# forestagostinelli/DeepCubeA

Hardware: AMD Instinct MI355X
Metric: A* nodes expanded/sec on cube3, batch 20k (higher is better)
Workload: dtype u8 states / f64 cost keys / f32 heuristic

## Files before the change

### deepcubea_amd/csrc/dca_engine.hip

```cpp
#include <string.h>

#include <new>
#include <vector>

#include "dca_common.h"
#include "dca_tile.h"

namespace dca {

constexpr int NBIN = 4096;
constexpr int kBinsPerThread = NBIN / 1024;
constexpr int kLgNbin = 12;
constexpr int kSub = 2048;
constexpr int kScanBlocks = 256;
constexpr int kCollectBlocks = 512;
constexpr int kRankBlocks = 256;
constexpr uint32_t kTinyBin = 512;
constexpr int kSortCap = 8192;
constexpr int RT = 512;
constexpr int kRegEnt = 16;
constexpr uint32_t kLdsEnt = RT * kRegEnt;
constexpr int kStash = 2560;
constexpr int kSegs = NBIN + 1 + kSub;
constexpr uint32_t kGiantBin = 8192;
// ... 1934 lines not shown
                s0[u] = S.off[sub];
                cn[u] = S.off[sub + 1] - s0[u];
                rank[u] = s0[u];
                if (!((livem >> u) & 1u)) cn[u] = 0;
                if (cn[u] > kSubMax && refinable) {
                    bigm |= 1u << u;
                    cn[u] = 0;
                }
                trip = cn[u] > trip ? cn[u] : trip;
            }
            for (uint32_t jj = 0; jj < trip; jj++) {
#pragma unroll
                for (int u = 0; u < U; u++) {
                    const uint32_t j = s0[u] + (jj < cn[u] ? jj : 0u);
                    const bool less = pair_less(LK[j], LI[j], o[u], id[u]);
                    rank[u] += (jj < cn[u] && less) ? 1u : 0u;
                }
            }
            uint32_t retm = 0;
#pragma unroll
            for (int u = 0; u < U; u++) {
                const uint32_t p = p0 + (uint32_t)u * RT + t;
                o[u] = idmode ? kbase : kbase + o[u];
                if ((bigm >> u) & 1u) {
                    K2[p] = o[u];
                    I2[p] = id[u];
                } else if ((livem >> u) & 1u) {
                    if (rank[u] < need) emit_pop(E, c, it.off + rank[u], o[u], id[u]);
                    else retm |= 1u << u;
                }
            }
            ret_put_many<U>(E, S, nf, n_ord, retm, o, id);
        }
        rank_push(S, it, tsub, need, refinable, lo_sub, in_hi);
        __syncthreads();
        prof_end(E, P_RB_ORDER);
        return;
    }
    {
        u128 vmin = ~(u128)0, vmax = 0;
        for (uint32_t b0 = 0; b0 < n; b0 += kLdsEnt) {
            uint64_t ek[kRegEnt];
            uint32_t ei[kRegEnt];
#pragma unroll
            for (int j = 0; j < kRegEnt; j++) {
                const uint32_t i = b0 + t + (uint32_t)RT * j, ic = i < n ? i : n - 1;
                ek[j] = K[ic];
                ei[j] = I[ic];
            }
#pragma unroll
            for (int j = 0; j < kRegEnt; j++)
                if (b0 + t + (uint32_t)RT * j < n) {
                    const u128 v = comp_of(ek[j], ei[j]);
                    vmin = v < vmin ? v : vmin;
                    vmax = v > vmax ? v : vmax;
                }
        }
        rank_range(S, vmin, vmax);
    }
    const u128 base = ((u128)S.vmin_hi << 64) | S.vmin_lo;
    const uint32_t bits = S.bits;
    if (lg > bits) lg = bits;
    const uint32_t nsub = 1u << lg, shc = bits - lg;
    for (uint32_t b0 = 0; b0 < n; b0 += kLdsEnt) {
        uint64_t ek[kRegEnt];
        uint32_t ei[kRegEnt];
#pragma unroll
        for (int j = 0; j < kRegEnt; j++) {
            const uint32_t i = b0 + t + (uint32_t)RT * j, ic = i < n ? i : n - 1;
            ek[j] = K[ic];
            ei[j] = I[ic];
        }
#pragma unroll
        for (int j = 0; j < kRegEnt; j++)
            if (b0 + t + (uint32_t)RT * j < n) atomicAdd(&S.cnt[sub_of(ek[j], ei[j], base, shc, nsub)], 1u);
    }
    __syncthreads();
    rank_prefix(S, nsub, need);
    const uint32_t tsub = S.tsub;
    const bool tsub_pushed = S.off[tsub + 1] - S.off[tsub] > kSubMax && shc > 0;
    ret_begin(c, S, nf, (n - S.off[tsub + 1]) + (tsub_pushed ? 0u : S.off[tsub + 1] - need));
    RetAcc acc{};
    const uint32_t n_ord_all = c->n_ord;
    for (uint32_t b0 = 0; b0 < n; b0 += kLdsEnt) {
        uint64_t ek[kRegEnt];
        uint32_t ei[kRegEnt];
#pragma unroll
        for (int j = 0; j < kRegEnt; j++) {
            const uint32_t i = b0 + t + (uint32_t)RT * j, ic = i < n ? i : n - 1;
            ek[j] = K[ic];
            ei[j] = I[ic];
        }
        uint32_t retm = 0;
#pragma unroll
        for (int j = 0; j < kRegEnt; j++) {
            const bool live = b0 + t + (uint32_t)RT * j < n;
            uint32_t sub = 0;
            if (live) {
                sub = sub_of(ek[j], ei[j], base, shc, nsub);
                if (sub <= tsub) {
                    const uint32_t p = S.off[sub] + atomicAdd(&S.cnt[sub], 1u);
                    K2[p] = ek[j];
                    I2[p] = ei[j];
                }
            }
            retm |= (live && sub > tsub ? 1u : 0u) << j;
        }
        ret_put_many<kRegEnt>(E, S, nf, n_ord_all, retm, ek, ei);
    }
    __syncthreads();
    const uint32_t m = S.off[tsub + 1];
    for (uint32_t p0 = 0; p0 < m; p0 += RT) {
        const uint32_t p = p0 + t;
        bool live = p < m;
        uint64_t k = 0;
        uint32_t id = 0, rank = 0;
        if (live) {
            k = K2[p];
            id = I2[p];
            const uint32_t sub = sub_of(k, id, base, shc, nsub);
            const uint32_t s0 = S.off[sub], e0 = S.off[sub + 1];
            if (e0 - s0 > kSubMax && shc > 0) {
                live = false;
            } else {
                rank = s0;
                for (uint32_t j = s0; j < e0; j++) rank += pair_less(K2[j], I2[j], k, id) ? 1u : 0u;
                if (rank < need) emit_pop(E, c, it.off + rank, k, id);
            }
        }
        ret_put(E, c, S, nf, live && rank >= need, k, id, acc);
    }
    rank_push(S, it, tsub, need, shc > 0);
    ret_end(c, nf, acc);
    __syncthreads();
}

__global__ __launch_bounds__(RT) void k_rank(const Eng* __restrict__ engs) {
    const Eng& E = engs[blockIdx.y];
    gp<Ctl> c = E.ctl;
    if (c->done) return;
    Stamp stamp(E, P_RANK);
    __shared__ RankShared S;
    extern __shared__ __attribute__((aligned(16))) uint8_t rank_lds[];
    uint64_t* LK = reinterpret_cast<uint64_t*>(rank_lds);
    uint32_t* LI = reinterpret_cast<uint32_t*>(rank_lds + (size_t)kLdsEnt * 8);
    const uint32_t t = threadIdx.x;
    const uint32_t nf = c->cur_f;
    const uint32_t tseg = c->tseg, want = c->want;
    const uint32_t n_big = c->n_big, n_ord = c->n_ord;
    if (blockIdx.x == gridDim.x - 1) {
        const uint32_t bstar = c->bstar, pre_b = c->pre_b, cn_star = c->cn_star;
        if (want != 0) {
            for (uint32_t bin = t; bin < bstar; bin += RT) E.hist[bin] = 0;
            if (t == 0) E.hist[bstar] = cn_star - (want - pre_b);
        }
        for (uint32_t i = t; i < (uint32_t)kSegs; i += RT) E.fill[i] = 0;
        if (c->giant)
            for (uint32_t i = t; i < (uint32_t)(kMaxLevels * kSub); i += RT) E.subhist[i] = 0;
    }
    {
        Stamp sub(E, P_RANK_SMALL);
        for (uint32_t p0 = blockIdx.x * RT; p0 < n_ord; p0 += gridDim.x * RT)
            rank_small_entries(E, c, S, LK, LI, nf, p0, n_ord, want);
    }
    Stamp sub2(E, P_RANK_BIG);
    for (uint32_t bi = (blockIdx.x + gridDim.x - 64u) % gridDim.x; bi < n_big; bi += gridDim.x) {
        const uint32_t unit = E.big_list[bi];
        const uint32_t f = unit & 0xFFFFu;
        const uint32_t o = E.pre[f], n = E.pre[f + 1] - o;
        __syncthreads();
        if (t == 0) {
            S.stack[0] = RankItem{o, n, (f == tseg) ? want - o : n, 0u, (unit >> 16) & 15u, unit >> 20, 0u};
            S.sp = 1;
            S.fail = 0;
        }
        for (;;) {
            __syncthreads();
            const uint32_t sp = S.sp;
            if (sp == 0 || sp > (uint32_t)kRankStack) break;
            const RankItem it = S.stack[sp - 1];
            __syncthreads();
            if (t == 0) S.sp = sp - 1;
            __syncthreads();
            rank_item(E, c, S, LK, LI, nf, want, it);
        }
        if (t == 0 && (S.fail || S.sp != 0)) c->failed = 1;
    }
}

__device__ __forceinline__ void close_pop(const Eng& E, gp<Ctl> c, const IterState& S0, uint32_t it, uint32_t want,
                                          uint32_t npop, uint32_t base, bool fail) {
    IterState N = S0;
    if (E.sem == DCA_SEM_PY) {
        const unsigned long long gb = c->goal_best;
        if (gb != ~0ull) {
            c->stop_after = 1;
            c->goal_id = E.pop_id[(uint32_t)(gb & 0xFFFFFFFFull)] & ID_MASK;
        }
    } else {
        const uint32_t fs = c->first_solved;
        if (fs != NIL) {
            const float cst = (float)cost_of_key(E.pop_key[fs]);
            if (E.B == 1) {
                N.best_id = E.pop_id[fs] & ID_MASK;
                N.best_cost = cst;
                N.has_best = 1;
                c->stop_after = 1;
            } else if (!S0.has_best || S0.best_cost > cst) {
                N.best_id = E.pop_id[fs] & ID_MASK;
                N.best_cost = cst;
                N.has_best = 1;
            }
        }
        if (S0.has_best && (float)cost_of_key(E.pop_key[0]) >= N.best_cost) c->stop_after = 1;
    }
    if (fail) {
        c->failed = 1;
        c->done = 1;
        c->front_dead.v -= want;
        return;
    }
    const uint32_t m = npop * (uint32_t)E.A;
    N.npop = npop;
    N.m = m;
    N.base = base;
    N.pool_n = base + m;
    c->S[(it + 1) & 1] = N;
    c->gen += (int64_t)m;
    c->expanded += npop;
}

constexpr uint8_t F_KEEP = 1, F_MIN = 2, F_NEW = 4;

template <int ENV, int DIM>
__device__ __forceinline__ uint32_t child_word_from_parent(uint32_t pw, uint32_t w, uint32_t a, const uint8_t* ltab) {
    using EV = EnvT<ENV, DIM>;
    const int gbase = (int)(threadIdx.x & 63u) & ~15;
    uint32_t out = 0;
    if constexpr (ENV == DCA_ENV_CUBE3) {
#pragma unroll
        for (uint32_t b = 0; b < 4; b++) {
            const uint32_t i = 4 * w + b;
            const uint32_t p = i < (uint32_t)EV::D ? ltab[a * EV::D + i] : 0u;
            const uint32_t v = (uint32_t)__shfl((int)pw, gbase + (int)(p >> 2));
            if (i < (uint32_t)EV::D) out |= ((v >> (8 * (p & 3))) & 0xFFu) << (8 * b);
        }
    } else if constexpr (ENV == DCA_ENV_LIGHTSOUT) {
#pragma unroll
        for (uint32_t b = 0; b < 4; b++) {
            const uint32_t i = 4 * w + b;
            if (i < (uint32_t)EV::D) {
                const uint32_t v = (pw >> (8 * b)) & 0xFFu;
                out |= (lightsout_flip(DIM, (int)a, (int)i) ? ((v + 1u) & 1u) : v) << (8 * b);
            }
        }
    } else {
        uint32_t z = 0xFFFFu;
#pragma unroll
        for (int b = 3; b >= 0; b--)
            if (4 * w + b < (uint32_t)EV::D && ((pw >> (8 * b)) & 0xFFu) == 0u) z = 4 * w + b;
        for (int o = 8; o > 0; o >>= 1) {
            const uint32_t y = (uint32_t)__shfl_xor((int)z, o);
            z = y < z ? y : z;
        }
        z = z < (uint32_t)EV::D ? z : 0u;
        const uint32_t sw = (uint32_t)npuzzle_swap(DIM, (int)z, (int)a);
#pragma unroll
        for (uint32_t b = 0; b < 4; b++) {
            const uint32_t i = 4 * w + b;
            const uint32_t src = i < (uint32_t)EV::D ? ((i == z) ? sw : i) : 0u;
            const uint32_t v = (uint32_t)__shfl((int)pw, gbase + (int)(src >> 2));
            if (i < (uint32_t)EV::D) out |= ((i == sw) ? 0u : ((v >> (8 * (src & 3))) & 0xFFu)) << (8 * b);
        }
    }
    return out;
}

constexpr int kEngTile = 16;
template <int ENV, int DIM, int OH>
__global__ __launch_bounds__(kThreads) void k_expand(const Eng* __restrict__ engs, int heur_id, int write_nn) {
    const Eng& E = engs[blockIdx.y];
    using EV = EnvT<ENV, DIM>;
    using TL = Tile<ENV, DIM, kEngTile>;
    constexpr int kTileParents = kEngTile;
    constexpr int TP = kEngTile;
    typedef uint32_t u32x4 __attribute__((ext_vector_type(4)));
    constexpr int kPermChunks = (int)sizeof(Cube3Perm) / 16;
    u32x4 permv;
    if constexpr (ENV == DCA_ENV_CUBE3) {
        static_assert(sizeof(Cube3Perm) % 16 == 0 && alignof(Cube3Perm) == 16 && TL::TAB_BYTES == (int)sizeof(Cube3Perm),
                      "cube3's move table is staged in 16-byte pieces");
        const u32x4* pp = reinterpret_cast<const u32x4*>(&d_cube3_perm) + min(threadIdx.x, (uint32_t)kPermChunks - 1u);
        asm volatile("global_load_dwordx4 %0, %1, off" : "=v"(permv) : "v"(pp) : "memory");
    }
    gp<Ctl> c = E.ctl;
    if (c->done) return;
    Stamp stamp(E, P_EXPAND);
    extern __shared__ __attribute__((aligned(16))) uint8_t smem[];
    uint8_t* lpar = smem;
    uint8_t* ltab = smem + TL::PAR_BYTES;
    uint8_t* lst = smem + TL::LDS_BYTES;
    __shared__ uint32_t l_pid[TP], l_g[TP], l_mv[TP];
    __shared__ uint32_t l_qn, l_qcc[kThreads], l_qrep[kThreads], l_qres[kThreads];
    __shared__ uint32_t l_ohq;
    const uint32_t it = (uint32_t)c->iters;
    const IterState S0 = c->S[it & 1];
    const uint32_t want = c->want;
    const uint32_t cur_new = c->cur_f;
    uint32_t npop = want;
    if (E.sem == DCA_SEM_CPP) {
        const uint32_t fs = c->first_solved;
        if (fs != NIL) npop = fs + 1;
    }
    const uint32_t base = (S0.pool_n + 15u) & ~15u;
    const bool fail = (uint64_t)base + (uint64_t)npop * (uint64_t)EV::A > (uint64_t)E.max_nodes;
    if (blockIdx.x == 0 && threadIdx.x == 0) close_pop(E, c, S0, it, want, npop, base, fail);
    if (fail) return;
    const uint32_t r0 = blockIdx.x * kTileParents;
    if (E.sem == DCA_SEM_CPP && r0 + kTileParents > npop) {
        uint32_t r = r0 + threadIdx.x;
        bool back = threadIdx.x < kTileParents && r >= npop && r < want;
        open_append(E, c, cur_new, back, back ? E.pop_key[r] : 0, back ? E.pop_id[r] : 0);
        if (back) atomicAdd(&E.hist[bin_of(E.pop_key[r], c->sel_kmin, c->shift)], 1u);
    }
    if (r0 >= npop) return;
    const uint32_t np = min((uint32_t)kTileParents, npop - r0);
    if (OH != 0 && threadIdx.x == 0) l_ohq = 0;
    {
        constexpr int WPR = (EV::D + 3) / 4;
        static_assert(WPR + 2 <= 16, "16 lanes per parent: the row's words, its path cost, its move");
        static_assert(TP * 16 == kThreads, "one 16-lane group per parent of the tile");
        const uint32_t w = threadIdx.x & 15, r = threadIdx.x >> 4;
        gp<const uint32_t> ppop = E.pop_id;
        gp<const uint8_t> pst = E.state, pg = reinterpret_cast<gp<const uint8_t>>(E.g), pmv = E.move;
        asm volatile("" : "+s"(ppop), "+s"(pst), "+s"(pg), "+s"(pmv));
        const uint32_t pid = ppop[r0 + min(r, np - 1u)] & ID_MASK;
        const GatherWord gw = gather_word(EV::D, (int)w);
        const bool row_lane = w < (uint32_t)WPR;
        gp<const uint8_t> src = (row_lane ? pst : pg) + (row_lane ? (size_t)pid * EV::D + (uint32_t)gw.off : (size_t)pid * 4);
        uint32_t v = load_word(src);
        uint32_t mv = pmv[pid];
        asm volatile("" : "+v"(v), "+v"(mv));
        if (r < np) {
            if (w < (uint32_t)WPR) {
                v >>= gw.shift;
                uint8_t* dst = lpar + r * EV::D + 4 * w;
                if constexpr (EV::D % 4 == 0) {
                    *reinterpret_cast<uint32_t*>(dst) = v;
                } else if constexpr (EV::D % 2 == 0) {
                    *reinterpret_cast<uint16_t*>(dst) = (uint16_t)v;
                    if (gw.n == 4) *reinterpret_cast<uint16_t*>(dst + 2) = (uint16_t)(v >> 16);
                } else {
#pragma unroll
                    for (int b = 0; b < 4; b++)
                        if (b < gw.n) dst[b] = (uint8_t)(v >> (8 * b));
                }
            } else if (w == (uint32_t)WPR) {
                l_pid[r] = pid;
                l_g[r] = v;
            } else if (w == (uint32_t)WPR + 1u) {
                l_mv[r] = mv;
            }
        }
    }
    if constexpr (ENV == DCA_ENV_CUBE3) {
        asm volatile("s_waitcnt vmcnt(0)" : "+v"(permv) : : "memory");
        if (threadIdx.x < (uint32_t)kPermChunks) reinterpret_cast<u32x4*>(ltab)[threadIdx.x] = permv;
    }
    __syncthreads();
    if constexpr (ENV != DCA_ENV_CUBE3) {
        stage_tables<ENV, DIM>(ltab, lpar, np);
        __syncthreads();
    }
    TL t{lpar, ltab};
    const uint32_t nchild = np * EV::A;
    const uint32_t j0 = r0 * EV::A;

    auto oh_emit = [&]() {
        if constexpr (OH != 0) {
            constexpr uint32_t ROW = EV::D * EV::DEPTH;
            constexpr uint32_t EPC = 16 / OH;
            const uint32_t te = nchild * ROW;
            const uint32_t one16 = E.oh_dtype == DCA_DT_F16 ? 0x3C00u : 0x3F80u;
            gp<uint8_t> goh = E.onehot + (size_t)j0 * ROW * OH;
            const uint32_t nch = (te + EPC - 1) / EPC;
            auto staged_nnet = [&](uint32_t i) -> uint32_t {
                const uint32_t b = lst[i];
                return ENV == DCA_ENV_CUBE3 ? (b * 57u) >> 9 : b;
            };
            for (;;) {
                uint32_t piece = 0;
                if ((threadIdx.x & 63u) == 0) piece = atomicAdd(&l_ohq, 1u);
                piece = (uint32_t)__builtin_amdgcn_readfirstlane((int)piece);
                if (piece * 64u >= nch) break;
                const uint32_t q = piece * 64u + (threadIdx.x & 63u);
                if (q >= nch) continue;
                uint32_t e0 = q * EPC;
                if constexpr (ENV == DCA_ENV_CUBE3 && OH == 4) {
                    if (e0 + EPC <= te) {
                        const uint32_t P0 = (q << 1) / 3u, phase = (q << 1) - 3u * P0;
                        uint32_t w[4];
                        cube3_onehot32_chunk(phase, staged_nnet(P0), phase == 2u ? staged_nnet(P0 + 1u) : 0u, w);
                        store16(goh + (size_t)e0 * OH, w, true);
                        continue;
                    }
                }
                if constexpr (ENV == DCA_ENV_CUBE3 && OH == 2) {
                    if (e0 + EPC <= te) {
                        const uint32_t P0 = (q << 2) / 3u, phase = (q << 2) - 3u * P0;
                        uint32_t w[4];
                        cube3_onehot16_chunk(phase, staged_nnet(P0), staged_nnet(P0 + 1u), one16, w);
                        store16(goh + (size_t)e0 * OH, w, true);
                        continue;
                    }
                }
                uint32_t cch = e0 / ROW, e = e0 - cch * ROW;
                uint32_t pos = e / EV::DEPTH, col = e - pos * EV::DEPTH;
                uint32_t r = cch / EV::A, a = cch - r * EV::A;
                uint32_t nb = staged_nnet(cch * EV::D + pos);
                uint32_t w[4] = {0, 0, 0, 0};
#pragma unroll
                for (uint32_t k = 0; k < EPC; k++) {
                    bool hot = (nb == col) && (e0 + k < te);
                    if constexpr (OH == 4)
                        w[k] = hot ? 0x3F800000u : 0u;
                    else
                        w[k >> 1] |= (hot ? one16 : 0u) << (16 * (k & 1));
                    if (++col == EV::DEPTH) {
                        col = 0;
                        if (++pos == EV::D) {
                            pos = 0;
                            if (++a == EV::A) {
                                a = 0;
                                ++r;
                            }
                        }
                        nb = staged_nnet((r * EV::A + a) * EV::D + pos);
                    }
                }
                uint8_t* dst = goh + (size_t)e0 * OH;
                if (e0 + EPC <= te) {
                    store16(dst, w, true);
                } else {
                    for (uint32_t k = 0; e0 + k < te; k++) {
                        if constexpr (OH == 4)
                            reinterpret_cast<uint32_t*>(dst)[k] = w[k];
                        else
                            reinterpret_cast<uint16_t*>(dst)[k] = (uint16_t)(w[k >> 1] >> (16 * (k & 1)));
                    }
                }
            }
        }
    };

    if (threadIdx.x == 0) l_qn = 0;
    for (uint32_t cc0 = 0; cc0 < nchild; cc0 += kThreads) {
        const uint32_t cc = cc0 + threadIdx.x;
        const bool cvalid = cc < nchild;
        uint64_t h = 0;
        uint64_t roww[(EV::D + 7) / 8];
        bool known = false;
        if (cvalid) {
        uint32_t r = cc / EV::A, a = cc - r * EV::A;
        static_assert((uint64_t)EV::D * 255u * (7u * (EV::D - 1) + 3u) < (1ull << 32), "the heuristics' byte sum overflows 32 bits");
        static_assert(7 * (EV::D - 1) + 3 < 65536, "the heuristics' weights are two bytes");
        uint32_t sum = 0, sum_hi = 0;
        h = hash_init(EV::D);
        uint32_t manh = 0;
        bool ok = true;
#pragma unroll
        for (int k = 0; k < EV::D; k += 8) {
            uint64_t w = 0;
#pragma unroll
            for (int j = 0; j < 8; j++) {
                if (k + j < EV::D) {
                    uint32_t b = t.child_byte(r, a, k + j);
                    w |= (uint64_t)b << (8 * j);
                    if constexpr (ENV == DCA_ENV_NPUZZLE) manh += manhattan_term(DIM, (uint32_t)(k + j), b);
                }
            }
            h = hash_word(h, w);
            roww[k >> 3] = w;
            ok &= (w & row_word_mask(EV::D, k >> 3)) == goal_word(ENV, EV::D, k >> 3);
#pragma unroll
            for (int q = 0; q < 8; q += 4) {
                if (k + q < EV::D) {
                    const uint32_t x = (uint32_t)(w >> (8 * q));
                    sum = __builtin_amdgcn_udot4(x, sum_weights(k + q, 0), sum, false);
                    if (sum_weights(k + q, 8) != 0u) sum_hi = __builtin_amdgcn_udot4(x, sum_weights(k + q, 8), sum_hi, false);
                }
            }
            uint8_t* dst = lst + cc * EV::D + k;
#pragma unroll
            for (int j = 0; j < 8; j += 2) {
                if (k + j + 1 < EV::D && (EV::D % 2) == 0) {
                    *reinterpret_cast<uint16_t*>(dst + j) = (uint16_t)(w >> (8 * j));
                } else {
                    if (k + j < EV::D) dst[j] = (uint8_t)(w >> (8 * j));
                    if (k + j + 1 < EV::D) dst[j + 1] = (uint8_t)(w >> (8 * j + 8));
                }
            }
        }
        h = hash_final(h);
        const uint32_t j = j0 + cc, id = base + j, pid = l_pid[r];
        const uint32_t gp = l_g[r];
        bool noop = false;
        if constexpr (ENV == DCA_ENV_NPUZZLE) noop = ltab[r * 8 + 1 + a] == ltab[r * 8];
        known = known_duplicate(ENV, gp, l_mv[r], a, noop);
        if (a == 0) E.pop_g[r0 + r] = gp;
        E.g[id] = (int32_t)(gp + 1u);
        E.parent[id] = pid;
        E.move[id] = (uint8_t)a;
        E.solved[id] = ok ? 1 : 0;
        if (heur_id >= 0) E.child_h[j] = heur_from(heur_id, (uint64_t)(sum + (sum_hi << 8)), h, manh);
        }
        {
            constexpr int NWD = (EV::D + 3) / 4;
            const uint32_t j = j0 + cc, id = base + j;
            const uint64_t tag = h >> 32;
            bool active = cvalid && !known, inserted = false, paused = false;
            uint32_t slot = (uint32_t)h & E.tab_mask, v0 = known ? 0u : GINF, rep_id = 0, probes = 0, qi = 0;
            __syncthreads();
            for (;;) {
                if (active && !paused) {
                    for (;;) {
                        const uint4 sl = *reinterpret_cast<const uint4*>(&E.tab[slot]);
                        uint64_t e = ((uint64_t)sl.y << 32) | sl.x;
                        v0 = sl.z;
                        if (e == EMPTY) {
                            const uint64_t old = atomicCAS((unsigned long long*)&E.tab[slot].entry, (unsigned long long)EMPTY,
                                                           (unsigned long long)((tag << 32) | id));
                            if (old == EMPTY) {
                                inserted = true;
                                active = false;
                                break;
                            }
                            e = old;
                        }
                        if ((e >> 32) == tag) {
                            const uint32_t rep = (uint32_t)e;
                            if (rep >= base) {
                                qi = atomicAdd(&l_qn, 1u);
                                l_qcc[qi] = cc;
                                l_qrep[qi] = rep;
                                paused = true;
                                break;
                            }
                            gp<const uint8_t> rrow = E.state + (size_t)rep * EV::D;
                            uint32_t diff = 0;
#pragma unroll
                            for (int k = 0; k < NWD; k++) {
                                uint32_t v = 0;
                                if (4 * k + 4 <= EV::D) {
                                    v = load_word(rrow + 4 * k);
                                } else {
                                    for (int b = 0; 4 * k + b < EV::D; b++) v |= (uint32_t)rrow[4 * k + b] << (8 * b);
                                }
                                diff |= v ^ (uint32_t)(roww[k >> 1] >> (32 * (k & 1)));
                            }
                            if (diff == 0) {
                                rep_id = rep;
                                active = false;
                                break;
                            }
                        }
                        slot = (slot + 1) & E.tab_mask;
                        if (++probes > E.tab_mask) {
                            c->failed = 1;
                            active = false;
                            break;
                        }
                    }
                }
                __syncthreads();
                const uint32_t nq = l_qn;
                if (nq == 0) break;
                for (uint32_t q0 = 0; q0 < nq; q0 += kThreads / 16) {
                    const uint32_t item = q0 + (threadIdx.x >> 4), w = threadIdx.x & 15u;
                    const bool iv = item < nq;
                    const uint32_t itc = iv ? item : 0u;
                    const uint32_t rrel = l_qrep[itc] - base;
                    const uint32_t rk = rrel / (uint32_t)EV::A, a2 = rrel - rk * (uint32_t)EV::A;
                    const uint32_t ppid = E.pop_id[rk] & ID_MASK;
                    gp<const uint8_t> prow = E.state + (size_t)ppid * EV::D;
                    uint32_t pw = 0;
                    if (w < (uint32_t)NWD) {
                        if (4 * w + 4 <= (uint32_t)EV::D) {
                            pw = load_word(prow + 4 * w);
                        } else {
                            for (uint32_t b = 0; 4 * w + b < (uint32_t)EV::D; b++) pw |= (uint32_t)prow[4 * w + b] << (8 * b);
                        }
                    }
                    const uint32_t cw = child_word_from_parent<ENV, DIM>(pw, w, a2, ltab);
                    const uint8_t* mrow = lst + l_qcc[itc] * EV::D;
                    uint32_t mv = 0;
                    for (uint32_t b = 0; b < 4 && 4 * w + b < (uint32_t)EV::D; b++) mv |= (uint32_t)mrow[4 * w + b] << (8 * b);
                    uint32_t diff = w < (uint32_t)NWD ? (cw ^ mv) : 0u;
                    for (int o = 8; o > 0; o >>= 1) diff |= (uint32_t)__shfl_xor((int)diff, o);
                    if (iv && w == 0) l_qres[item] = diff == 0 ? 1u : 0u;
                }
                __syncthreads();
                if (paused) {
                    paused = false;
                    if (l_qres[qi]) {
                        rep_id = l_qrep[qi];
                        active = false;
                    } else {
                        slot = (slot + 1) & E.tab_mask;
                        probes++;
                    }
                }
                __syncthreads();
                if (threadIdx.x == 0) l_qn = 0;
                __syncthreads();
            }
            if (cvalid) {
                uint32_t prev = NIL;
                if (!inserted && !known) {
                    const uint32_t old_head = atomicExch(&E.tab[slot].head, id);
                    if (old_head >= base)
                        prev = old_head - base;
                    else if (rep_id >= base)
                        prev = rep_id - base;
                }
                E.child_next[j] = prev;
                E.child_slot[j] = slot;
                E.child_v0[j] = v0;
                E.child_flags[j] = inserted ? F_NEW : 0;
                if (prev != NIL) {
                    E.child_multi[j] = 1;
                    E.child_multi[prev] = 1;
                }
            }
        }
    }

    __syncthreads();
    if (!write_nn) {
        const uint32_t tb = nchild * EV::D;
        gp<uint8_t> gpool = E.state + ((size_t)base + j0) * EV::D;
        const uint32_t nfull = tb >> 4;
        for (uint32_t q = threadIdx.x; q < nfull; q += kThreads)
            reinterpret_cast<uint4*>(gpool)[q] = reinterpret_cast<const uint4*>(lst)[q];
#pragma unroll 1
        for (uint32_t bq = (nfull << 4) + threadIdx.x; bq < tb; bq += kThreads) gpool[bq] = lst[bq];
    } else {
        const uint32_t tb = nchild * EV::D;
        gp<uint8_t> gpool = E.state + ((size_t)base + j0) * EV::D;
        gp<uint8_t> gnn = E.nnet_in + (size_t)j0 * EV::D;
        const uint32_t nfull = tb >> 4;
        for (uint32_t q = threadIdx.x; q < nfull; q += kThreads) {
            const uint4 v = reinterpret_cast<const uint4*>(lst)[q];
            reinterpret_cast<uint4*>(gpool)[q] = v;
            if constexpr (ENV == DCA_ENV_CUBE3) {
                auto div9 = [](uint32_t x) {
                    uint32_t lo = (((x & 0x00FF00FFu) * 57u) >> 9) & 0x00070007u;
                    uint32_t hi = ((((x >> 8) & 0x00FF00FFu) * 57u) >> 9) & 0x00070007u;
                    return lo | (hi << 8);
                };
                reinterpret_cast<uint4*>(gnn)[q] = make_uint4(div9(v.x), div9(v.y), div9(v.z), div9(v.w));
            } else {
                reinterpret_cast<uint4*>(gnn)[q] = v;
            }
        }
#pragma unroll 1
        for (uint32_t bq = (nfull << 4) + threadIdx.x; bq < tb; bq += kThreads) {
            const uint32_t b = lst[bq];
            gpool[bq] = (uint8_t)b;
            gnn[bq] = (uint8_t)(ENV == DCA_ENV_CUBE3 ? (b * 57u) >> 9 : b);
        }
    }

    oh_emit();
}

struct Dec {
    bool keep, is_min;
    uint32_t first;
};
__device__ __forceinline__ Dec decide_child(const Eng& E, uint32_t base, uint32_t m, uint32_t j, uint32_t slot,
                                            uint32_t v0, uint32_t gj, bool multi) {
    if (!multi) return Dec{gj < v0, true, j};
    bool dominated = false;
    uint32_t gmin = GINF, pmin = NIL, first = j;
    const uint32_t A = (uint32_t)E.A;
    uint32_t steps = 0;
    for (uint32_t k = E.tab[slot].head - base; k < m && steps <= m; k = E.child_next[k], steps++) {
        const uint32_t gk = E.pop_g[k / A] + 1u;
        dominated |= (k < j && gk <= gj);
        if (gk < gmin || (gk == gmin && k < pmin)) {
            gmin = gk;
            pmin = k;
        }
        first = k < first ? k : first;
    }
    return Dec{(gj < v0) && !dominated, j == pmin, first};
}

__device__ __forceinline__ void fix_representative(const Eng& E, uint32_t base, uint32_t slot, uint32_t id) {
    const uint64_t e = E.tab[slot].entry;
    if ((uint32_t)e >= base && (uint32_t)e != id) E.tab[slot].entry = (e & 0xFFFFFFFF00000000ull) | id;
}

__global__ __launch_bounds__(256) void k_decide(const Eng* __restrict__ engs) {
    const Eng& E = engs[blockIdx.y];
    gp<Ctl> c = E.ctl;
    if (c->done) return;
    Stamp stamp(E, P_DECIDE);
    const uint32_t j = blockIdx.x * 256 + threadIdx.x;
    gr<const IterState> S1 = st_next(c);
    const uint32_t m = S1.m, base = S1.base;
    if (j >= m) return;
    const uint32_t slot = E.child_slot[j];
    const bool multi = E.child_multi[j] != 0;
    const uint32_t gj = E.pop_g[j / (uint32_t)E.A] + 1u;
    const Dec d = decide_child(E, base, m, j, slot, E.child_v0[j], gj, multi);
    E.child_flags[j] = (E.child_flags[j] & F_NEW) | (d.keep ? F_KEEP : 0) | (d.is_min ? F_MIN : 0);
    if (multi && j == d.first) fix_representative(E, base, slot, base + j);
}

template <int ENV, int DIM, int OH>
__global__ __launch_bounds__(256) void k_pack(const Eng* __restrict__ engs) {
    const Eng& E = engs[blockIdx.y];
    using EV = EnvT<ENV, DIM>;
    gp<Ctl> c = E.ctl;
    if (c->done) {
        if (blockIdx.x == 0 && threadIdx.x == 0) {
            atomicAdd(&E.pk_n[1], 1u);
            if (c->failed) atomicAdd(&E.pk_n[2], 1u);
        }
        return;
    }
    Stamp stamp(E, P_PACK);
    const uint32_t m = st_next(c).m, base = st_next(c).base;
    if (blockIdx.x * 256 >= m) return;
    __shared__ uint32_t sh[6];
    __shared__ uint32_t lsrc[256];
    __shared__ __attribute__((aligned(16))) uint8_t lrow[256 * EV::D];
    const uint32_t j = blockIdx.x * 256 + threadIdx.x;
    const bool keep = j < m && (E.child_flags[j] & F_KEEP);
    const int lane = threadIdx.x & 63, wv = threadIdx.x >> 6;
    const unsigned long long mask = __ballot(keep);
    if (lane == 0) sh[wv] = (uint32_t)__popcll(mask);
    __syncthreads();
    if (threadIdx.x == 0) {
        uint32_t tot = 0;
        for (int w = 0; w < 4; w++) {
            uint32_t t = sh[w];
            sh[w] = tot;
            tot += t;
        }
        sh[4] = tot;
        sh[5] = tot ? atomicAdd(E.pk_n, tot) : 0u;
    }
    __syncthreads();
    const uint32_t total = sh[4], gbase = sh[5];
    const uint32_t lr = sh[wv] + (uint32_t)__popcll(mask & ((1ull << lane) - 1ull));
    if (j < m) E.kept_pos[j] = keep ? gbase + lr : NIL;
    if (keep) lsrc[lr] = j;
    __syncthreads();
    if (total == 0) return;
    if (threadIdx.x < total) E.pk_src[gbase + threadIdx.x] = E.inst * E.M + lsrc[threadIdx.x];
    const uint32_t tb = total * EV::D;
    for (uint32_t q = threadIdx.x; q < tb; q += 256) {
        const uint32_t r = q / EV::D, b = q - r * EV::D;
        const uint32_t v = E.state[(size_t)(base + lsrc[r]) * EV::D + b];
        lrow[q] = (uint8_t)(ENV == DCA_ENV_CUBE3 ? (v * 57u) >> 9 : v);
    }
    __syncthreads();
    gp<uint8_t> gnn = E.pk_nnet + (size_t)gbase * EV::D;
    for (uint32_t q = threadIdx.x; q < tb; q += 256) gnn[q] = lrow[q];
    if constexpr (OH != 0) {
        constexpr uint32_t ROW = EV::D * EV::DEPTH, EPC = 16 / OH;
        const uint32_t cpr = E.pk_stride / EPC;
        const uint32_t one16 = E.pk_dtype == DCA_DT_F16 ? 0x3C00u : 0x3F80u;
        uint4* goh = reinterpret_cast<uint4*>(E.pk_onehot + (size_t)gbase * E.pk_stride * OH);
        const uint32_t nch = total * cpr;
        for (uint32_t q = threadIdx.x; q < nch; q += 256) {
            const uint32_t r = q / cpr, e0 = (q - r * cpr) * EPC;
            uint32_t pos = e0 / EV::DEPTH, col = e0 - pos * EV::DEPTH;
            uint32_t nb = pos < (uint32_t)EV::D ? lrow[r * EV::D + pos] : 0xFFFFu;
            uint32_t w[4] = {0, 0, 0, 0};
#pragma unroll
            for (uint32_t k = 0; k < EPC; k++) {
                const bool hot = (e0 + k < ROW) && nb == col;
                if constexpr (OH == 4)
                    w[k] = hot ? 0x3F800000u : 0u;
                else
                    w[k >> 1] |= (hot ? one16 : 0u) << (16 * (k & 1));
                if (++col == EV::DEPTH) {
                    col = 0;
                    ++pos;
                    nb = pos < (uint32_t)EV::D ? lrow[r * EV::D + pos] : 0xFFFFu;
                }
            }
            goh[q] = make_uint4(w[0], w[1], w[2], w[3]);
        }
    }
}

__device__ __forceinline__ void commit_ticket(const Eng& E, gp<Ctl> c) {
    __syncthreads();
    if (threadIdx.x == 0) {
        uint32_t t = atomicAdd(&c->ticket_a.v, 1u);
        if (t == gridDim.x - 1) {
            c->ticket_a.v = 0;
            c->iters += 1;
            if (c->stop_after || c->failed) {
                c->done = 1;
            } else {
                const uint32_t fb = c->cur_f;
                const uint32_t live = __hip_atomic_load(&c->open_n[fb].v, __ATOMIC_RELAXED, __HIP_MEMORY_SCOPE_AGENT) -
                                      __hip_atomic_load(&c->front_dead.v, __ATOMIC_RELAXED, __HIP_MEMORY_SCOPE_AGENT) - c->front_above;
                c->want = live < (uint32_t)E.B ? live : (uint32_t)E.B;
                c->ret_n.v = 0;
                c->goal_best = ~0ull;
                c->first_solved = NIL;
                c->gbar.v = 0;
                c->grange.kmin = ~0ull;
                c->grange.kmax = 0;
                c->grange.imin = ~0u;
                c->grange.imax = 0;
            }
        }
    }
// ... 1158 lines not shown
```

### deepcubea_amd/csrc/dca_tile.h

```cpp
#pragma once
#include "dca_common.h"

namespace dca {

constexpr int kTileParents = 64;
constexpr int kThreads = 256;

template <int ENV, int DIM>
struct EnvT;
template <>
struct EnvT<DCA_ENV_CUBE3, 0> {
    static constexpr int D = 54, A = 12, DEPTH = 6;
};
template <int DIM>
struct EnvT<DCA_ENV_NPUZZLE, DIM> {
    static constexpr int D = DIM * DIM, A = 4, DEPTH = DIM * DIM;
};

template <>
struct EnvT<DCA_ENV_CUBE4, 0> {
    static constexpr int D = 96, A = 24, DEPTH = 6;
};

template <int DIM>
struct EnvT<DCA_ENV_LIGHTSOUT, DIM> {
    static constexpr int D = DIM * DIM, A = DIM * DIM, DEPTH = 6;
};

struct GatherWord {
    int off, shift, n;
};
constexpr __host__ __device__ inline GatherWord gather_word(int D, int w) {
    if (4 * w >= D) return GatherWord{0, 0, 0};
    if (4 * w + 4 <= D) return GatherWord{4 * w, 0, 4};
    return GatherWord{D - 4, 8 * (4 * w + 4 - D), D - 4 * w};
}
constexpr bool gather_covers(int D) {
    if (D < 4 || (D + 3) / 4 + 2 > 16) return false;
    int seen[64] = {};
    for (int w = 0; w < 16; w++) {
        const GatherWord g = gather_word(D, w);
        if (g.n == 0) continue;
        if (g.off < 0 || g.off + 4 > D || g.shift != 8 * (4 - g.n)) return false;
        for (int b = 0; b < g.n; b++) {
            const int src = g.off + g.shift / 8 + b;
            if (src != 4 * w + b || src >= D) return false;
            seen[src]++;
        }
    }
    for (int i = 0; i < D; i++)
        if (seen[i] != 1) return false;
    return true;
}
static_assert(gather_covers(9) && gather_covers(16) && gather_covers(25) && gather_covers(36) && gather_covers(49) &&
                  gather_covers(54),
              "parent gather: the lanes' dwords must cover each row byte exactly once and none outside the row");

template <int ENV, int DIM, int TP = kTileParents>
struct Tile {
    using E = EnvT<ENV, DIM>;
    static constexpr int PAR_BYTES = ((TP * E::D + 15) / 16) * 16;
    static constexpr int TAB_BYTES = ENV == DCA_ENV_CUBE3 ? ((12 * 54 + 15) / 16) * 16
                                     : ENV == DCA_ENV_CUBE4 ? 24 * 96 : ENV == DCA_ENV_NPUZZLE ? TP * 8 : 16;
    static constexpr int LDS_BYTES = PAR_BYTES + TAB_BYTES + 16 + 256;

    const uint8_t* par;
    const uint8_t* tab;

    __device__ __forceinline__ uint32_t child_byte(uint32_t r, uint32_t a, uint32_t i) const {
        if constexpr (ENV == DCA_ENV_CUBE3 || ENV == DCA_ENV_CUBE4) {
            return par[r * E::D + tab[a * E::D + i]];
        } else if constexpr (ENV == DCA_ENV_LIGHTSOUT) {
            const uint32_t v = par[r * E::D + i];
            return lightsout_flip(DIM, (int)a, (int)i) ? ((v + 1u) & 1u) : v;
        } else {
            uint32_t z = tab[r * 8];
            uint32_t s = tab[r * 8 + 1 + a];
            uint32_t src = (i == z) ? s : i;
            uint32_t v = par[r * E::D + src];
            return (i == s) ? 0u : v;
        }
    }
    __device__ __forceinline__ uint32_t nnet_byte(uint32_t r, uint32_t a, uint32_t i) const {
        uint32_t b = child_byte(r, a, i);
        if constexpr (ENV == DCA_ENV_CUBE3) return (b * 57u) >> 9;
        return b;
    }
};

static __constant__ Cube3Perm d_cube3_perm = make_cube3_perm();
static __constant__ Cube4Perm d_cube4_perm = make_cube4_perm();

__device__ __forceinline__ void stage_tile(uint8_t* lds, const uint8_t* __restrict__ g, uint32_t nbytes, bool aligned) {
    if (aligned) {
        uint32_t nch = nbytes >> 4;
        for (uint32_t q = threadIdx.x; q < nch; q += kThreads)
            reinterpret_cast<uint4*>(lds)[q] = reinterpret_cast<const uint4*>(g)[q];
        for (uint32_t b = (nch << 4) + threadIdx.x; b < nbytes; b += kThreads) lds[b] = g[b];
    } else {
        for (uint32_t b = threadIdx.x; b < nbytes; b += kThreads) lds[b] = g[b];
    }
}

template <int ENV, int DIM>
__device__ __forceinline__ void stage_tables(uint8_t* tab, const uint8_t* par, uint32_t np) {
    using E = EnvT<ENV, DIM>;
    if constexpr (ENV == DCA_ENV_CUBE3) {
        for (uint32_t i = threadIdx.x; i < 12 * 54; i += kThreads) tab[i] = d_cube3_perm.p[i / 54][i % 54];
    } else if constexpr (ENV == DCA_ENV_CUBE4) {
        for (uint32_t i = threadIdx.x; i < 24 * 96; i += kThreads) tab[i] = d_cube4_perm.p[i / 96][i % 96];
    } else if constexpr (ENV == DCA_ENV_LIGHTSOUT) {
    } else {
        for (uint32_t r = threadIdx.x; r < np; r += kThreads) {
            uint32_t z = 0;
            for (int i = E::D - 1; i >= 0; i--)
                if (par[r * E::D + i] == 0) z = (uint32_t)i;
            tab[r * 8] = (uint8_t)z;
            for (int a = 0; a < 4; a++) tab[r * 8 + 1 + a] = (uint8_t)npuzzle_swap(DIM, (int)z, a);
        }
    }
}

__device__ __forceinline__ void cube3_onehot16_chunk(uint32_t phase, uint32_t v0, uint32_t v1, uint32_t one16, uint32_t (&w)[4]) {
    const uint32_t s0 = (v0 & 1u) ? (one16 << 16) : one16, k0 = v0 >> 1;
    const uint32_t s1 = (v1 & 1u) ? (one16 << 16) : one16, k1 = v1 >> 1;
    const uint32_t a0 = k0 == 0u ? s0 : 0u, a1 = k0 == 1u ? s0 : 0u, a2 = k0 == 2u ? s0 : 0u;
    const uint32_t b0 = k1 == 0u ? s1 : 0u, b1 = k1 == 1u ? s1 : 0u, b2 = k1 == 2u ? s1 : 0u;
    w[0] = phase == 0u ? a0 : phase == 1u ? a1 : a2;
    w[1] = phase == 0u ? a1 : phase == 1u ? a2 : b0;
    w[2] = phase == 0u ? a2 : phase == 1u ? b0 : b1;
    w[3] = phase == 0u ? b0 : phase == 1u ? b1 : b2;
}

__device__ __forceinline__ void cube3_onehot32_chunk(uint32_t phase, uint32_t v0, uint32_t v1, uint32_t (&w)[4]) {
    const uint32_t a = v0 - 2u * phase;
    const uint32_t b = phase == 2u ? v1 : a - 2u;
    w[0] = a == 0u ? 0x3F800000u : 0u;
    w[1] = a == 1u ? 0x3F800000u : 0u;
    w[2] = b == 0u ? 0x3F800000u : 0u;
    w[3] = b == 1u ? 0x3F800000u : 0u;
}

__device__ __forceinline__ void store16(uint8_t* dst, const uint32_t (&w)[4], bool aligned) {
    if (aligned) {
        *reinterpret_cast<uint4*>(dst) = make_uint4(w[0], w[1], w[2], w[3]);
    } else {
#pragma unroll
        for (int k = 0; k < 16; k++) dst[k] = (uint8_t)(w[k >> 2] >> (8 * (k & 3)));
    }
}


}
```

Before: 104.8 million.

## Build cube3 children with compile-time byte-permute words and stage child writes through LDS

For cube3, each thread now builds its child state from the parent's packed words with compile-time byte-permute (v_perm) sequences specialised per move. This replaces 54 LDS byte lookups through the move table. Threads are remapped so each wave handles three fixed moves across 16 parents, which keeps the move index wave-uniform and lets the switch on move pick one specialised path. Child metadata (g, parent, move, solved, heuristic) is buffered in LDS and written by threads in child order so the global stores coalesce. The cost is extra shared memory, an added LDS round trip, and larger code from the unrolled per-move specialisations.

```diff
diff --git a/deepcubea_amd/csrc/dca_engine.hip b/deepcubea_amd/csrc/dca_engine.hip
--- a/deepcubea_amd/csrc/dca_engine.hip
+++ b/deepcubea_amd/csrc/dca_engine.hip
@@ -2260,6 +2260,8 @@
     uint8_t* lst = smem + TL::LDS_BYTES;
     __shared__ uint32_t l_pid[TP], l_g[TP], l_mv[TP];
     __shared__ uint32_t l_qn, l_qcc[kThreads], l_qrep[kThreads], l_qres[kThreads];
+    __shared__ float l_h[ENV == DCA_ENV_CUBE3 ? TP * EV::A : 1];
+    __shared__ uint8_t l_ok[ENV == DCA_ENV_CUBE3 ? TP * EV::A : 1];
     __shared__ uint32_t l_ohq;
     const uint32_t it = (uint32_t)c->iters;
     const IterState S0 = c->S[it & 1];
@@ -2413,13 +2415,42 @@
 
     if (threadIdx.x == 0) l_qn = 0;
     for (uint32_t cc0 = 0; cc0 < nchild; cc0 += kThreads) {
-        const uint32_t cc = cc0 + threadIdx.x;
-        const bool cvalid = cc < nchild;
+        uint32_t cc = cc0 + threadIdx.x;
+        bool cvalid = cc < nchild;
+        uint32_t cw[ENV == DCA_ENV_CUBE3 ? 14 : 1], r3 = 0, a3 = 0;
+        if constexpr (ENV == DCA_ENV_CUBE3) {
+            static_assert(TP == 16 && EV::A == 12 && EV::D == 54 && TP * EV::A <= kThreads, "cube3: 16 parents x 12 moves, one round");
+            const uint32_t m = (threadIdx.x >> 4) & 3u;
+            const uint32_t wave = (uint32_t)__builtin_amdgcn_readfirstlane((int)(threadIdx.x >> 6));
+            const uint32_t r = r3 = threadIdx.x & 15u;
+            a3 = 3u * wave + m;
+            cc = r * EV::A + a3;
+            cvalid = m < 3u && r < np;
+            uint32_t pw[14];
+            __builtin_memcpy(pw, lpar + r * EV::D, 52);
+            pw[13] = *reinterpret_cast<const uint16_t*>(lpar + r * EV::D + 52);
+            auto build3 = [&](auto a0) {
+                constexpr int A0 = decltype(a0)::value;
+                if (m == 0u)
+                    cube3_child_words<A0>(pw, cw);
+                else if (m == 1u)
+                    cube3_child_words<A0 + 1>(pw, cw);
+                else
+                    cube3_child_words<A0 + 2>(pw, cw);
+            };
+            switch (wave) {
+                case 0: build3(std::integral_constant<int, 0>{}); break;
+                case 1: build3(std::integral_constant<int, 3>{}); break;
+                case 2: build3(std::integral_constant<int, 6>{}); break;
+                default: build3(std::integral_constant<int, 9>{}); break;
+            }
+        }
         uint64_t h = 0;
         uint64_t roww[(EV::D + 7) / 8];
         bool known = false;
         if (cvalid) {
         uint32_t r = cc / EV::A, a = cc - r * EV::A;
+        if constexpr (ENV == DCA_ENV_CUBE3) r = r3, a = a3;
         static_assert((uint64_t)EV::D * 255u * (7u * (EV::D - 1) + 3u) < (1ull << 32), "the heuristics' byte sum overflows 32 bits");
         static_assert(7 * (EV::D - 1) + 3 < 65536, "the heuristics' weights are two bytes");
         uint32_t sum = 0, sum_hi = 0;
@@ -2429,12 +2460,16 @@
 #pragma unroll
         for (int k = 0; k < EV::D; k += 8) {
             uint64_t w = 0;
-#pragma unroll
-            for (int j = 0; j < 8; j++) {
-                if (k + j < EV::D) {
-                    uint32_t b = t.child_byte(r, a, k + j);
-                    w |= (uint64_t)b << (8 * j);
-                    if constexpr (ENV == DCA_ENV_NPUZZLE) manh += manhattan_term(DIM, (uint32_t)(k + j), b);
+            if constexpr (ENV == DCA_ENV_CUBE3) {
+                w = (uint64_t)cw[k >> 2] | ((uint64_t)cw[(k >> 2) + 1] << 32);
+            } else {
+#pragma unroll
+                for (int j = 0; j < 8; j++) {
+                    if (k + j < EV::D) {
+                        uint32_t b = t.child_byte(r, a, k + j);
+                        w |= (uint64_t)b << (8 * j);
+                        if constexpr (ENV == DCA_ENV_NPUZZLE) manh += manhattan_term(DIM, (uint32_t)(k + j), b);
+                    }
                 }
             }
             h = hash_word(h, w);
@@ -2466,11 +2501,16 @@
         if constexpr (ENV == DCA_ENV_NPUZZLE) noop = ltab[r * 8 + 1 + a] == ltab[r * 8];
         known = known_duplicate(ENV, gp, l_mv[r], a, noop);
         if (a == 0) E.pop_g[r0 + r] = gp;
+        if constexpr (ENV == DCA_ENV_CUBE3) {
+            l_ok[cc] = ok ? 1 : 0;
+            if (heur_id >= 0) l_h[cc] = heur_from(heur_id, (uint64_t)(sum + (sum_hi << 8)), h, manh);
+        } else {
         E.g[id] = (int32_t)(gp + 1u);
         E.parent[id] = pid;
         E.move[id] = (uint8_t)a;
         E.solved[id] = ok ? 1 : 0;
         if (heur_id >= 0) E.child_h[j] = heur_from(heur_id, (uint64_t)(sum + (sum_hi << 8)), h, manh);
+        }
         }
         {
             constexpr int NWD = (EV::D + 3) / 4;
@@ -2479,6 +2519,17 @@
             bool active = cvalid && !known, inserted = false, paused = false;
             uint32_t slot = (uint32_t)h & E.tab_mask, v0 = known ? 0u : GINF, rep_id = 0, probes = 0, qi = 0;
             __syncthreads();
+            if constexpr (ENV == DCA_ENV_CUBE3) {
+                const uint32_t c2 = threadIdx.x;
+                if (c2 < nchild) {
+                    const uint32_t r2 = c2 / EV::A, a2 = c2 - r2 * EV::A, j2 = j0 + c2, id2 = base + j2;
+                    E.g[id2] = (int32_t)(l_g[r2] + 1u);
+                    E.parent[id2] = l_pid[r2];
+                    E.move[id2] = (uint8_t)a2;
+                    E.solved[id2] = l_ok[c2];
+                    if (heur_id >= 0) E.child_h[j2] = l_h[c2];
+                }
+            }
             for (;;) {
                 if (active && !paused) {
                     for (;;) {
diff --git a/deepcubea_amd/csrc/dca_tile.h b/deepcubea_amd/csrc/dca_tile.h
--- a/deepcubea_amd/csrc/dca_tile.h
+++ b/deepcubea_amd/csrc/dca_tile.h
@@ -1,4 +1,6 @@
 #pragma once
+#include <utility>
+
 #include "dca_common.h"
 
 namespace dca {
@@ -88,6 +90,85 @@
     }
 };
 
+
+constexpr __host__ __device__ inline uint32_t perm_bytes(uint32_t hi, uint32_t lo, uint32_t sel) {
+#if defined(__HIP_DEVICE_COMPILE__)
+    if (!__builtin_is_constant_evaluated()) return __builtin_amdgcn_perm(hi, lo, sel);
+#endif
+    uint32_t out = 0;
+    for (int b = 0; b < 4; b++) {
+        const uint32_t s = (sel >> (8 * b)) & 0xFFu;
+        const uint32_t v = s < 4u ? (lo >> (8 * s)) & 0xFFu : s < 8u ? (hi >> (8 * (s - 4u))) & 0xFFu : 0u;
+        out |= v << (8 * b);
+    }
+    return out;
+}
+
+struct Cube3WordPlan {
+    bool copy;
+    int n, src[4];
+    uint32_t sel[3];
+};
+constexpr Cube3WordPlan cube3_word_plan(int a, int w) {
+    constexpr int D = 54;
+    Cube3WordPlan p{true, 0, {0, 0, 0, 0}, {0, 0, 0}};
+    int which[4] = {-1, -1, -1, -1}, byte[4] = {0, 0, 0, 0};
+    for (int b = 0; b < 4; b++) {
+        const int i = 4 * w + b;
+        if (i >= D) continue;
+        const int s = kCube3Perm.p[a][i];
+        if (s != i) p.copy = false;
+        int k = 0;
+        while (k < p.n && p.src[k] != s / 4) k++;
+        if (k == p.n) p.src[p.n++] = s / 4;
+        which[b] = k;
+        byte[b] = s % 4;
+    }
+    for (int b = 0; b < 4; b++) {
+        p.sel[0] |= (which[b] == 0 ? (uint32_t)byte[b] : which[b] == 1 ? 4u + (uint32_t)byte[b] : 0x0Cu) << (8 * b);
+        for (int k = 2; k < 4; k++) p.sel[k - 1] |= (which[b] == k ? 4u + (uint32_t)byte[b] : (uint32_t)b) << (8 * b);
+    }
+    return p;
+}
+
+template <int A, int W>
+constexpr __host__ __device__ inline uint32_t cube3_child_word(const uint32_t (&pw)[14]) {
+    constexpr Cube3WordPlan p = cube3_word_plan(A, W);
+    if constexpr (p.copy) {
+        return pw[W];
+    } else {
+        uint32_t acc = perm_bytes(pw[p.src[p.n > 1 ? 1 : 0]], pw[p.src[0]], p.sel[0]);
+        if constexpr (p.n > 2) acc = perm_bytes(pw[p.src[2]], acc, p.sel[1]);
+        if constexpr (p.n > 3) acc = perm_bytes(pw[p.src[3]], acc, p.sel[2]);
+        return acc;
+    }
+}
+template <int A, int... W>
+constexpr __host__ __device__ inline void cube3_child_words_seq(const uint32_t (&pw)[14], uint32_t (&cw)[14],
+                                                                std::integer_sequence<int, W...>) {
+    ((cw[W] = cube3_child_word<A, W>(pw)), ...);
+}
+template <int A>
+constexpr __host__ __device__ inline void cube3_child_words(const uint32_t (&pw)[14], uint32_t (&cw)[14]) {
+    static_assert(A >= 0 && A < 12, "cube3 has 12 moves");
+    cube3_child_words_seq<A>(pw, cw, std::make_integer_sequence<int, 14>{});
+}
+template <int A>
+constexpr bool cube3_child_words_match() {
+    uint32_t pw[14] = {}, cw[14] = {};
+    for (int i = 0; i < 54; i++) pw[i >> 2] |= (uint32_t)i << (8 * (i & 3));
+    cube3_child_words<A>(pw, cw);
+    for (int i = 0; i < 56; i++)
+        if (((cw[i >> 2] >> (8 * (i & 3))) & 0xFFu) != (i < 54 ? (uint32_t)kCube3Perm.p[A][i] : 0u)) return false;
+    return true;
+}
+template <int... A>
+constexpr bool cube3_child_words_match_all(std::integer_sequence<int, A...>) {
+    return (cube3_child_words_match<A>() && ...);
+}
+static_assert(cube3_child_words_match_all(std::make_integer_sequence<int, 12>{}),
+              "cube3_child_words<A> must apply kCube3Perm.p[A] for every move A");
+
 static __constant__ Cube3Perm d_cube3_perm = make_cube3_perm();
 static __constant__ Cube4Perm d_cube4_perm = make_cube4_perm();
 
```

Measured after the change: 105.9 million, median of 6. 1.01x the previous value.
